# Graphegon/pygraphblas

Measured on AMD Instinct MI355X. Metric: GFLOPS + GB/s (vs roofline) for mxv/mxm on R-MAT-22, 1/2/4/8 GPU, higher is better.
Workload: dtype f64; 1 GPU; R-MAT scale-22 FP64 PLUS_TIMES SpMV (GrB_mxv), edgefactor 16, BASELINE.json configs[1]; n=4194304, nnz=65245211, semiring=PLUS_TIMES_FP64, parallelism=rowblock1, transport=none (one GPU), device=AMD Radeon Graphics gfx950:sramecc+:xnack-

## Files before the change

### pygraphblas_amd/csrc/grb_spmv_xcd.hpp

```cpp
#pragma once
#include "grb_spmv_tiles.hpp"
#include "grb_matops.hpp"

namespace grb {

constexpr int XP = 8;
constexpr int XPMAX = 64;
constexpr uint32_t XP_RB = 1024;
constexpr int XP_CT = 512;
constexpr uint32_t XP_UNIT = 16384;
constexpr int XP_ST = 512;
constexpr int XP_SW = XP_ST / 64;

struct XcdPlan {
  DevBuf hot_cols;
  DevBuf pcol, pval;
  DevBuf trow;
  DevBuf col16, extras, tinfo;
  uint64_t ncold = 0;
  DevBuf lrow;
  DevBuf blockptr;
  DevBuf m_bstart;
  DevBuf m_blockptr;
  DevBuf m_slot;
// ... 264 lines not shown
    const uint2 hh = *(const uint2*)(col16 + q0);
    const uint32_t h[2] = {hh.x, hh.y};
    uint32_t before = 0, nc = 0;
    for (int u = 0; u < 4; u++) {
      const uint32_t w = (h[u >> 1] >> (16 * (u & 1))) & 0x7FFFu; const bool cold = w >= H;
      const unsigned long long m = __ballot(cold);
      before += __builtin_amdgcn_mbcnt_hi((uint32_t)(m >> 32), __builtin_amdgcn_mbcnt_lo((uint32_t)m, 0u)); nc += cold ? 1u : 0u;
    }
    const uint32_t xr = tinfo[2 * (size_t)g + 1] + before;
    uint32_t x0 = 0, x1 = 0, x2 = 0;
    if (nc) { const uint32_t* xp = (const uint32_t*)extras + (xr >> 1); x0 = xp[0]; x1 = xp[1]; x2 = xp[2]; }
    const uint64_t wa = ((uint64_t)x1 << 32) | x0, wb = ((uint64_t)x2 << 32) | x1;
    uint32_t q = xr & 1u;
    for (int u = 0; u < 4; u++) {
      const uint32_t w16 = (h[u >> 1] >> (16 * (u & 1))) & 0xFFFFu, code = w16 & 0x7FFFu, flag = (w16 & 0x8000u) << 16;
      const bool cold = code >= H;
      const uint32_t lo = (uint32_t)((q < 2u ? wa >> (16u * q) : wb >> (16u * (q - 2u)))) & 0xFFFFu;
      const uint32_t c = flag | (cold ? XT_COLD | (((code - H) << 16) | lo) : code);
      q += cold ? 1u : 0u;
      if (c != pcol[q0 + u]) { const unsigned long long n = atomicAdd(bad, 1ull); if (n == 0) { bad[1] = q0 + u; bad[2] = ((unsigned long long)c << 32) | pcol[q0 + u]; } }
    }
    if (lane == 0 && tinfo[2 * (size_t)g] != trow[g]) atomicAdd(bad + 3, 1ull);
  }
}
template <class T> __global__ __launch_bounds__(256) void k_xp_hot_gather(const T* __restrict__ u, const uint32_t* __restrict__ hot_cols, uint32_t total, T* __restrict__ xhot) {
  for (uint32_t i = (blockIdx.x * 256 + threadIdx.x) * 4u; i < total; i += gridDim.x * 1024u) {
    if (i + 4u <= total) {
      const uint4 c = *(const uint4*)(hot_cols + i);
      const T x0 = u[c.x], x1 = u[c.y], x2 = u[c.z], x3 = u[c.w];
      xhot[i] = x0; xhot[i + 1] = x1; xhot[i + 2] = x2; xhot[i + 3] = x3;
    } else for (uint32_t j = i; j < total; j++) xhot[j] = u[hot_cols[j]];
  }
}
constexpr uint32_t XP_CONT = 0x8000u, XP_HEAD = 0x4000u, XP_LROW = 0x07FFu;
static_assert(XP_RB <= XP_LROW + 1, "row id inside a block and the two flags share 16 bits");
static __global__ void k_xp_cont_flags(const uint32_t* __restrict__ subrow_row, const uint32_t* __restrict__ vfirst, uint16_t* __restrict__ lrow) {
  uint32_t pb[XP + 1];
#pragma unroll
  for (int k = 0; k <= XP; k++) pb[k] = vfirst[k];
  const uint32_t F = pb[XP];
  for (uint32_t s = blockIdx.x * 256 + threadIdx.x; s < F; s += gridDim.x * 256) {
    const uint32_t r = subrow_row[s];
    bool first = false, last = s + 1 == F;
#pragma unroll
    for (int k = 0; k <= XP; k++) { first = first || pb[k] == s; last = last || pb[k] == s + 1; }
    const bool cont = !first && subrow_row[s - 1] == r, more = !last && subrow_row[s + 1] == r;
    lrow[s] = (uint16_t)((r % XP_RB) | (cont ? XP_CONT : 0u) | (!cont && more ? XP_HEAD : 0u));
  }
}
constexpr int XP_NA = 2;
template <class T, class SR>
__global__ __launch_bounds__(XP_CT) void k_xp_combine(uint32_t nrows, const uint32_t* __restrict__ blockptr, const uint16_t* __restrict__ subrow_lrow, const T* __restrict__ partial,
                                                      T* __restrict__ y, uint8_t* __restrict__ ypres, const SR sr) {
  __shared__ T acc[XP_NA][XP_RB];
  __shared__ uint8_t has[XP_NA][XP_RB];
  __shared__ T cval[2][XP_NA][XP_CT];
  __shared__ uint8_t ccont[2][XP_NA][XP_CT + 1];
  const uint32_t b = blockIdx.x, r0 = b * XP_RB, tid = threadIdx.x;
  for (uint32_t i = tid; i < XP_NA * XP_RB; i += XP_CT) (&has[0][0])[i] = 0;
  if (tid < 2 * XP_NA) ccont[tid / XP_NA][tid % XP_NA][XP_CT] = 0;
  uint32_t lo[XP], hi[XP], longest = 0;
#pragma unroll
  for (int k = 0; k < XP; k++) { lo[k] = blockptr[b * XP + k]; hi[k] = blockptr[(b + 1) * XP + k]; longest = hi[k] - lo[k] > longest ? hi[k] - lo[k] : longest; }
  for (uint32_t base = 0; base < longest; base += XP_CT) {
    uint32_t w[XP]; T v[XP];
#pragma unroll
    for (int k = 0; k < XP; k++) {
      const uint32_t s = lo[k] + base + tid; const bool ok = s < hi[k];
      w[k] = ok ? (uint32_t)subrow_lrow[s] : XP_CONT; v[k] = ok ? partial[s] : T();
    }
#pragma unroll
    for (int k0 = 0; k0 < XP; k0 += XP_NA) {
      const int buf = (k0 / XP_NA) & 1;
#pragma unroll
      for (int j = 0; j < XP_NA; j++) {
        const int k = k0 + j;
        const bool cont = (w[k] & XP_CONT) != 0 && lo[k] + base + tid < hi[k];
        ccont[buf][j][tid] = cont ? 1 : 0;
        if (cont) cval[buf][j][tid] = v[k];
      }
      __syncthreads();
#pragma unroll
      for (int j = 0; j < XP_NA; j++) {
        const int k = k0 + j;
        if (!(w[k] & XP_CONT)) {
          const uint32_t r = w[k] & XP_LROW; T x = v[k];
          const bool h = has[j][r] != 0; const T a = acc[j][r];
          if (w[k] & XP_HEAD) {
            uint32_t q = tid + 1;
            while (ccont[buf][j][q]) { x = sr.add(x, cval[buf][j][q]); q++; }
            if (q == XP_CT) for (uint32_t g = lo[k] + base + XP_CT; g < hi[k] && (subrow_lrow[g] & XP_CONT); g++) x = sr.add(x, partial[g]);
          }
          acc[j][r] = h ? sr.add(a, x) : x; has[j][r] = 1;
        }
      }
    }
    __syncthreads();
  }
  __syncthreads();
  for (uint32_t i = tid; i < XP_RB; i += XP_CT) {
    const uint32_t r = r0 + i;
    if (r < nrows) {
      bool h = has[0][i] != 0; T x = acc[0][i];
#pragma unroll
      for (int j = 1; j < XP_NA; j++) { const bool hj = has[j][i] != 0; const T xj = acc[j][i]; x = h ? (hj ? sr.add(x, xj) : x) : xj; h = h || hj; }
      y[r] = h ? x : T(); ypres[r] = h ? 1 : 0;
    }
  }
}

constexpr uint32_t XM_ROWS = 1024, XM_TARGET = 2048, XM_SLOTS = 2560;
constexpr int XM_CT = 256;
#ifndef XM_INFL
#define XM_INFL 4
#endif
static __global__ void k_xm_iota(uint32_t* p, uint64_t n) { for (uint64_t i = blockIdx.x * 256ull + threadIdx.x; i < n; i += gridDim.x * 256ull) p[i] = (uint32_t)i; }
static __global__ void k_xm_weights(const uint32_t* __restrict__ cnt, uint32_t nrows, uint32_t perrow, uint32_t* __restrict__ w) {
  for (uint32_t r = blockIdx.x * 256 + threadIdx.x; r <= nrows; r += gridDim.x * 256) w[r] = r < nrows ? cnt[r] + perrow : 0u;
}
static __global__ void k_xm_newblock(const uint32_t* __restrict__ P, uint32_t nrows, uint32_t target, uint32_t* __restrict__ f) {
  for (uint32_t r = blockIdx.x * 256 + threadIdx.x; r <= nrows; r += gridDim.x * 256) f[r] = r < nrows && (r == 0 || P[r] / target != P[r - 1] / target) ? 1u : 0u;
}
static __global__ void k_xm_bstart(const uint32_t* __restrict__ f, const uint32_t* __restrict__ fscan, uint32_t nrows, uint32_t nblocks, uint32_t* __restrict__ bstart) {
  for (uint32_t r = blockIdx.x * 256 + threadIdx.x; r <= nrows; r += gridDim.x * 256) { if (r == nrows) bstart[nblocks] = nrows; else if (f[r]) bstart[fscan[r]] = r; }
}
static __global__ void k_xm_rowoff(const uint32_t* __restrict__ f, const uint32_t* __restrict__ fscan, const uint32_t* __restrict__ bstart, const uint32_t* __restrict__ rfirst, uint32_t nrows,
                                   uint16_t* __restrict__ rowoff) {
  for (uint32_t r = blockIdx.x * 256 + threadIdx.x; r < nrows; r += gridDim.x * 256) { const uint32_t b = fscan[r] + f[r] - 1; rowoff[r] = (uint16_t)(rfirst[r] - rfirst[bstart[b]]); }
}
static __global__ void k_xm_slots(const uint32_t* __restrict__ skey, const uint32_t* __restrict__ sidx, uint64_t F, const uint32_t* __restrict__ f, const uint32_t* __restrict__ fscan,
                                  const uint32_t* __restrict__ bstart, const uint32_t* __restrict__ rfirst, uint16_t* __restrict__ slot) {
  for (uint64_t i = blockIdx.x * 256ull + threadIdx.x; i < F; i += gridDim.x * 256ull) { const uint32_t r = skey[i], b = fscan[r] + f[r] - 1; slot[sidx[i]] = (uint16_t)((uint32_t)i - rfirst[bstart[b]]); }
}
static __global__ void k_xm_block_starts(const uint32_t* __restrict__ subrow_row, const uint32_t* __restrict__ bstart, uint32_t nblocks, const uint32_t* __restrict__ vfirst, uint32_t np,
                                         uint32_t* __restrict__ blockptr) {
  for (uint32_t t = blockIdx.x * 256 + threadIdx.x; t < (nblocks + 1) * np; t += gridDim.x * 256) {
    const uint32_t b = t / np, k = t % np; const uint32_t target = bstart[b];
    uint32_t lo = vfirst[k], hi = vfirst[k + 1];
    while (lo < hi) { const uint32_t mid = lo + ((hi - lo) >> 1); if (subrow_row[mid] < target) lo = mid + 1; else hi = mid; }
    blockptr[t] = lo;
  }
}
static __global__ void k_xm_max(const uint32_t* __restrict__ cnt, uint32_t nrows, uint32_t* __restrict__ out) {
  __shared__ uint32_t s_m;
  if (threadIdx.x == 0) s_m = 0;
  __syncthreads();
  uint32_t m = 0;
  for (uint32_t r = blockIdx.x * 256 + threadIdx.x; r < nrows; r += gridDim.x * 256) m = cnt[r] > m ? cnt[r] : m;
  m = __builtin_amdgcn_wave_reduce_max_u32(m, 0);
  if ((threadIdx.x & 63) == 0 && m) atomicMax(&s_m, m);
  __syncthreads();
  if (threadIdx.x == 0 && s_m) atomicMax(out, s_m);
}
template <class T, class SR, int EPI = 0>
__global__ __launch_bounds__(XM_CT) void k_xp_merge(uint32_t nrows, uint32_t nblocks, const uint32_t* __restrict__ bstart, const uint32_t* __restrict__ blockptr, const uint16_t* __restrict__ slot,
                                                    const uint16_t* __restrict__ rowoff, const T* __restrict__ partial, T* __restrict__ y, uint8_t* __restrict__ ypres, const SR sr, const T fill = T()) {
  extern __shared__ __attribute__((aligned(16))) unsigned char xm_lds[];
  T* const vals = (T*)xm_lds;
  const uint32_t per = gridDim.x / XP, b = (blockIdx.x & (XP - 1)) * per + (blockIdx.x >> 3);
  const uint32_t tid = threadIdx.x;
  if (b >= nblocks) return;
  const uint32_t r0 = bstart[b], r1 = bstart[b + 1];
  uint32_t lo[XP], pre[XP + 1];
  pre[0] = 0;
#pragma unroll
  for (int k = 0; k < XP; k++) { lo[k] = blockptr[b * XP + k]; pre[k + 1] = pre[k] + (blockptr[(b + 1) * XP + k] - lo[k]); }
  const uint32_t total = pre[XP];
  for (uint32_t t0 = tid; t0 < total; t0 += XM_INFL * XM_CT) {
    T v[XM_INFL]; uint32_t sl[XM_INFL];
#pragma unroll
    for (int u = 0; u < XM_INFL; u++) {
      const uint32_t t = t0 + u * XM_CT; const bool ok = t < total;
      uint32_t s = 0;
#pragma unroll
      for (int k = 0; k < XP; k++) if (t >= pre[k] && t < pre[k + 1]) s = lo[k] + (t - pre[k]);
      v[u] = ok ? partial[s] : T(); sl[u] = ok ? (uint32_t)slot[s] : 0xFFFFFFFFu;
    }
#pragma unroll
    for (int u = 0; u < XM_INFL; u++) if (sl[u] != 0xFFFFFFFFu) vals[sl[u]] = v[u];
  }
  __syncthreads();
  const int lane = tid & 63;
  const uint32_t nr = r1 - r0, nround = (nr + XM_CT - 1) / XM_CT * XM_CT;
  for (uint32_t i = tid; i < nround; i += XM_CT) {
    const bool live = i < nr;
    const uint32_t r = r0 + i;
    const uint32_t o0 = live ? (uint32_t)rowoff[r] : 0u, o1 = live ? (i + 1 < nr ? (uint32_t)rowoff[r + 1] : total) : 0u;
    const bool wide = o1 - o0 > 64u;
    T acc = T();
    if (o1 > o0 && !wide) { acc = vals[o0]; for (uint32_t q = o0 + 1; q < o1; q++) acc = sr.add(acc, vals[q]); }
    unsigned long long todo = __ballot(wide);
    while (todo) {
      const int L = __builtin_ctzll(todo); todo &= todo - 1;
      const uint32_t q0 = (uint32_t)__shfl((int)o0, L, 64), q1 = (uint32_t)__shfl((int)o1, L, 64);
      T part = sr.identity; bool has = false;
      for (uint32_t q = q0 + lane; q < q1; q += 64) { part = has ? sr.add(part, vals[q]) : vals[q]; has = true; }
      const T red = wave_reduce_op<T, false>(sr.add_op(), has ? part : sr.identity);
      if (lane == L) acc = red;
    }
    if constexpr (EPI == 0) { if (live) { y[r] = acc; ypres[r] = o1 > o0 ? 1 : 0; } }
    else if constexpr (EPI == 1) { if (live && o1 > o0) y[r] = sr.add(y[r], acc); }
    else if constexpr (EPI == 2) { if (live) { y[r] = o1 > o0 ? sr.add(fill, acc) : fill; ypres[r] = 1; } }
    else {
      if constexpr (std::is_arithmetic<T>::value) {
        if (live && o1 > o0 && (sr.add_op() == B_MIN ? acc < fill : acc > fill)) { if (ypres[r]) y[r] = sr.add(y[r], acc); else { y[r] = acc; ypres[r] = 1; } }
      }
    }
  }
}

#ifndef XMW_TARGET_V
#define XMW_TARGET_V 4096
#endif
constexpr uint32_t XMW_TARGET = XMW_TARGET_V, XMW_ROWS = XMW_TARGET_V / 2;
constexpr int XMW_RPT = XMW_ROWS / XM_CT;
template <class T, class SR, int EPI = 0>
__global__ __launch_bounds__(XM_CT) void k_xp_merge_wide(uint32_t nrows, uint32_t nblocks, const uint32_t* __restrict__ bstart, const uint32_t* __restrict__ blockptr, const uint16_t* __restrict__ slot,
                                                         const uint16_t* __restrict__ rowoff, const T* __restrict__ partial, T* __restrict__ y, uint8_t* __restrict__ ypres, const SR sr, const T fill,
                                                         const uint32_t np, const uint32_t m_slots) {
  extern __shared__ __attribute__((aligned(16))) unsigned char xm_lds[];
  T* const vals = (T*)xm_lds;
  uint8_t* const flag = xm_lds + (size_t)m_slots * sizeof(T);
  __shared__ uint32_t s_lo[XPMAX], s_pre[XPMAX + 1];
  __shared__ T s_tsum[XM_CT];
  __shared__ uint8_t s_hasflag[XM_CT];
  const uint32_t per = (nblocks + XP - 1) / XP, tid = threadIdx.x, stride = gridDim.x >> 3;
  auto block_of = [&](uint32_t bb) -> uint32_t { const uint32_t b = (blockIdx.x & (XP - 1)) * per + bb; return bb < per && b < nblocks ? b : 0xFFFFFFFFu; };
  uint32_t bb = blockIdx.x >> 3, b = block_of(bb);
  uint32_t n_r0 = 0, n_r1 = 0, n_l0 = 0, n_len = 0;
  auto fetch_bounds = [&](uint32_t bn) __attribute__((always_inline)) {
    if (bn == 0xFFFFFFFFu) return;
    n_r0 = bstart[bn]; n_r1 = bstart[bn + 1];
    if (tid < np) { n_l0 = blockptr[bn * np + tid]; n_len = blockptr[(bn + 1) * np + tid] - n_l0; }
  };
  fetch_bounds(b);
  for (; b != 0xFFFFFFFFu; ) {
  __syncthreads();
  const uint32_t r0 = n_r0, r1 = n_r1, nr = r1 - r0;
  if (tid < 64u) {
    const bool in = tid < np;
    const uint32_t l0 = in ? n_l0 : 0u, len = in ? n_len : 0u;
    uint32_t incl = len;
#pragma unroll
    for (int d = 1; d < 64; d <<= 1) { const uint32_t o = (uint32_t)__shfl_up((int)incl, d, 64); if ((int)tid >= d) incl += o; }
    s_lo[tid] = l0; s_pre[tid] = in ? incl - len : 0xFFFFFFFFu;
    if (tid == 63u) { if (np < 64u) s_pre[np] = incl; s_pre[XPMAX] = np < 64u ? 0xFFFFFFFFu : incl; }
  }
  for (uint32_t q = tid * 4u; q < m_slots; q += XM_CT * 4u) *(uint32_t*)(flag + q) = 0u;
  uint32_t o0[XMW_RPT], o1[XMW_RPT];
#pragma unroll
  for (int j = 0; j < XMW_RPT; j++) {
    const uint32_t i = tid + (uint32_t)j * XM_CT; const bool live = i < nr;
    o0[j] = live ? (uint32_t)rowoff[r0 + i] : 0u;
    o1[j] = live && i + 1 < nr ? (uint32_t)rowoff[r0 + i + 1] : 0u;
  }
  __syncthreads();
  const uint32_t total = s_pre[np];
  bb += stride; const uint32_t b_next = block_of(bb);
  fetch_bounds(b_next);
  auto run_of = [&](uint32_t t) __attribute__((always_inline)) -> uint32_t {
    uint32_t k = 0;
#pragma unroll
    for (uint32_t step = 32u; step; step >>= 1) { const uint32_t cand = k + step; k = s_pre[cand] <= t ? cand : k; }
    return k;
  };
  for (uint32_t base = 0; base < total; base += 2u * XM_CT * 4u) {
    T v[2][4]; uint32_t sl[2][4];
#pragma unroll
    for (int g = 0; g < 2; g++) {
      const uint32_t t = base + (tid + (uint32_t)g * XM_CT) * 4u;
      uint32_t src[4]; bool ok[4];
      uint32_t k = t < total ? run_of(t) : 0u;
      uint32_t base = s_lo[k] - s_pre[k], end = s_pre[k + 1];
#pragma unroll
      for (int e = 0; e < 4; e++) {
        const uint32_t te = t + (uint32_t)e; ok[e] = te < total;
        while (ok[e] && te >= end) { k++; base = s_lo[k] - s_pre[k]; end = s_pre[k + 1]; }
        src[e] = ok[e] ? base + te : 0u;
      }
#pragma unroll
      for (int e = 0; e < 4; e++) { v[g][e] = ok[e] ? partial[src[e]] : T(); sl[g][e] = ok[e] ? (uint32_t)slot[src[e]] : 0xFFFFFFFFu; }
    }
#pragma unroll
    for (int g = 0; g < 2; g++)
#pragma unroll
      for (int e = 0; e < 4; e++) if (sl[g][e] != 0xFFFFFFFFu) vals[sl[g][e]] = v[g][e];
  }
#pragma unroll
  for (int j = 0; j < XMW_RPT; j++) {
    const uint32_t i = tid + (uint32_t)j * XM_CT;
    if (i < nr && i + 1 == nr) o1[j] = total;
    if (i < nr && o1[j] > o0[j]) flag[o0[j]] = 1;
  }
  __syncthreads();
  const uint32_t chunk = ((total + XM_CT - 1) / XM_CT) | 1u;
  const uint32_t q0 = tid * chunk < total ? tid * chunk : total, q1 = q0 + chunk < total ? q0 + chunk : total;
  uint32_t first = WP_NONE;
  {
    T acc = sr.identity;
    for (uint32_t q = q0; q < q1; q++) {
      const T v = vals[q]; const bool f = flag[q] != 0;
      acc = f ? v : sr.add(acc, v);
      vals[q] = acc;
      first = f && first == WP_NONE ? q : first;
    }
    s_tsum[tid] = acc; s_hasflag[tid] = first != WP_NONE ? 1 : 0;
  }
  __syncthreads();
  {
    const uint32_t lead_end = first != WP_NONE ? first : q1;
    const bool ends_row = lead_end == total || flag[lead_end < total ? lead_end : 0u] != 0;
    if (q1 > q0 && first != q0 && ends_row) {
      T c = sr.identity;
      for (uint32_t t = tid; t > 0;) { t--; c = sr.add(s_tsum[t], c); if (s_hasflag[t]) break; }
      vals[lead_end - 1u] = sr.add(c, vals[lead_end - 1u]);
    }
  }
  __syncthreads();
#pragma unroll
  for (int j = 0; j < XMW_RPT; j++) {
    const uint32_t i = tid + (uint32_t)j * XM_CT;
    if (i < nr) {
      const uint32_t r = r0 + i;
      const bool has = o1[j] > o0[j]; const T acc = has ? vals[o1[j] - 1u] : T();
      if constexpr (EPI == 0) { y[r] = acc; ypres[r] = has ? 1 : 0; }
      else if constexpr (EPI == 1) { if (has) y[r] = sr.add(y[r], acc); }
      else if constexpr (EPI == 2) { y[r] = has ? sr.add(fill, acc) : fill; ypres[r] = 1; }
      else {
        if constexpr (std::is_arithmetic<T>::value) {
          if (has && (sr.add_op() == B_MIN ? acc < fill : acc > fill)) { if (ypres[r]) y[r] = sr.add(y[r], acc); else { y[r] = acc; ypres[r] = 1; } }
        }
      }
    }
  }
  b = b_next;
  }
}

struct XtVariant { int depth, waves, exp; };
inline XtVariant xt_variant() {
  XtVariant v{XT_DEPTH, XT_WAVES, 0};
#ifdef XT_VARIANTS
  const char* e = getenv("GRB_MI355X_XT");
  if (e) { int d = v.depth, w = v.waves, x = 0; if (sscanf(e, "d%dw%de%d", &d, &w, &x) >= 2) { v.depth = d; v.waves = w; v.exp = x; } }
#endif
  return v;
}

template <class T> int xp_subpanels(uint64_t ncols, bool* forced_out) {
  const uint32_t forced = wp_env("GRB_MI355X_XS", 0);
  *forced_out = forced == 1 || forced == 2 || forced == 4 || forced == 8;
  if (*forced_out) return (int)forced;
  if (sizeof(T) <= 4 && ncols >= (1ull << 25)) return 8;
  if (ncols >= (1ull << 24)) return 4;
  if (sizeof(T) <= 4 && ncols >= (1ull << 23)) return 2;
  return 1;
}
static __global__ void k_xp_neg(const uint32_t* __restrict__ cnt, uint32_t n, uint32_t* __restrict__ key) {
// ... 224 lines not shown
    }
    gr.cbase[NS] = nchunks;
    DevBuf lc(((size_t)nchunks + 1) * 4), cstep(((size_t)nchunks + 1) * 4), pk((XPMAX + 2) * 4);
    GRB_HIP(hipMemsetAsync(lc.as<uint32_t>() + nchunks, 0, 4, stream()));
    { unsigned nb = (nchunks + 3) / 4; if (nb < 1) nb = 1; if (nb > 16384) nb = 16384;
      hipLaunchKernelGGL(k_sell_lc, dim3(nb), dim3(256), 0, stream(), sorted.as<uint32_t>(), plen.as<uint32_t>(), gr, nchunks, lc.as<uint32_t>()); }
    exclusive_scan_u32(lc.as<uint32_t>(), cstep.as<uint32_t>(), (uint64_t)nchunks + 1);
    hipLaunchKernelGGL(k_sell_pick, dim3(1), dim3(128), 0, stream(), cstep.as<uint32_t>(), gr, pk.as<uint32_t>());
    uint32_t hs[XPMAX + 2];
    GRB_HIP(hipMemcpyAsync(hs, pk.p, (NS + 1) * 4, hipMemcpyDeviceToHost, stream())); GRB_HIP(hipStreamSynchronize(stream()));
    const uint64_t nsteps = hs[NS];
    if (nsteps && nsteps * 256ull < (1ull << 40)) {
      P->s_nsteps = nsteps; P->s_nchunks = nchunks;
      P->s_col.alloc(nsteps * 256 + 64); P->s_perm.alloc((size_t)nchunks * 256 + 64);
      GRB_HIP(hipMemsetAsync(P->s_col.p, 0, nsteps * 256 + 64, stream())); GRB_HIP(hipMemsetAsync(P->s_perm.p, 0xFF, (size_t)nchunks * 256 + 64, stream()));
      if (with_vals) { P->s_val.alloc(nsteps * 64 * sizeof(T) + 64); GRB_HIP(hipMemsetAsync(P->s_val.p, 0, nsteps * 64 * sizeof(T) + 64, stream())); }
      hipLaunchKernelGGL(k_sell_inv, dim3(grid_n(F)), dim3(256), 0, stream(), sorted.as<uint32_t>(), F, inv.as<uint32_t>());
      hipLaunchKernelGGL((k_sell_scatter<T>), dim3(tile_grid), dim3(256), 0, stream(), P->pcol.as<uint32_t>(), with_vals ? P->pval.as<T>() : (const T*)nullptr, E.as<uint32_t>(), pstart.as<uint32_t>(),
                         inv.as<uint32_t>(), lc.as<uint32_t>(), cstep.as<uint32_t>(), sst, gr, ntiles, P->s_col.as<uint32_t>(), with_vals ? P->s_val.as<T>() : (T*)nullptr, P->s_perm.as<uint32_t>());
      { unsigned nb = (nchunks + 3) / 4; if (nb < 1) nb = 1; if (nb > 16384) nb = 16384;
        hipLaunchKernelGGL(k_sell_meta, dim3(nb), dim3(256), 0, stream(), P->s_col.as<uint32_t>(), lc.as<uint32_t>(), cstep.as<uint32_t>(), gr, nchunks); }
      uint32_t ibase[XPMAX + 1], nitems = 0;
      for (uint32_t k = 0; k < NS; k++) { ibase[k] = nitems; nitems += (hs[k + 1] - hs[k] + SELL_ITEM - 1) / SELL_ITEM; }
      ibase[NS] = nitems; P->s_nitems = nitems;
      DevBuf dib((XPMAX + 1) * 4);
      GRB_HIP(hipMemcpyAsync(dib.p, ibase, (NS + 1) * 4, hipMemcpyHostToDevice, stream()));
      P->s_items.alloc(((size_t)nitems + 2) * 4);
      hipLaunchKernelGGL(k_sell_items, dim3(grid_n((uint64_t)nitems + 1)), dim3(256), 0, stream(), cstep.as<uint32_t>(), gr, dib.as<uint32_t>(), nitems, (uint32_t)nsteps, P->s_items.as<uint32_t>());
      memcpy(sell_hs, hs, sizeof(uint32_t) * (NS + 1)); memcpy(sell_ib, ibase, sizeof(uint32_t) * (NS + 1));
      GRB_HIP(hipStreamSynchronize(stream()));
      P->sell = true;
      if (getenv("GRB_MI355X_VERBOSE")) fprintf(stderr, "[grb] lane-per-piece layout: %llu pieces in %u chunks, %llu steps = %.3f x the entries, %u work items\n", (unsigned long long)F, nchunks,
                                                (unsigned long long)nsteps, (double)nsteps * 64.0 / (double)nnz, nitems);
    }
  }
  constexpr bool c16 = xt_fmt<T>::C16;
  const bool keep32 = !c16 || wp_env("GRB_MI355X_XT_KEEP32", 0) != 0;
  if (c16) {
    DevBuf tcnt(((size_t)ntiles + 1) * 4), tcold(((size_t)ntiles + 1) * 4);
    GRB_HIP(hipMemsetAsync(tcnt.as<uint32_t>() + ntiles, 0, 4, stream()));
    unsigned nb = (ntiles + 3) / 4; if (nb < 1) nb = 1; if (nb > 16384) nb = 16384;
    hipLaunchKernelGGL(k_xc_count, dim3(nb), dim3(256), 0, stream(), P->pcol.as<uint32_t>(), ntiles, H, tcnt.as<uint32_t>());
    exclusive_scan_u32(tcnt.as<uint32_t>(), tcold.as<uint32_t>(), (uint64_t)ntiles + 1);
    uint32_t nc32 = 0;
    GRB_HIP(hipMemcpyAsync(&nc32, tcold.as<uint32_t>() + ntiles, 4, hipMemcpyDeviceToHost, stream())); GRB_HIP(hipStreamSynchronize(stream()));
    P->ncold = nc32;
    P->col16.alloc(nstore * 2); P->extras.alloc(P->ncold * 2 + 32); P->tinfo.alloc(((size_t)ntiles + 1) * 8);
    hipLaunchKernelGGL(k_xc_pack, dim3(nb), dim3(256), 0, stream(), P->pcol.as<uint32_t>(), P->trow.as<uint32_t>(), tcold.as<uint32_t>(), ntiles, H, P->col16.as<uint16_t>(), P->extras.as<uint16_t>(),
                       P->tinfo.as<uint32_t>());
    if (wp_env("GRB_MI355X_XC_VERIFY", 0)) {
      DevBuf bad(64); GRB_HIP(hipMemsetAsync(bad.p, 0, 64, stream()));
      hipLaunchKernelGGL(k_xc_verify, dim3(nb), dim3(256), 0, stream(), P->pcol.as<uint32_t>(), P->col16.as<uint16_t>(), P->extras.as<uint16_t>(), P->tinfo.as<uint32_t>(), P->trow.as<uint32_t>(), ntiles, H,
                         (unsigned long long*)bad.p);
      unsigned long long hb[4]; GRB_HIP(hipMemcpyAsync(hb, bad.p, 32, hipMemcpyDeviceToHost, stream())); GRB_HIP(hipStreamSynchronize(stream()));
      fprintf(stderr, "[grb] 16-bit column plane check: %llu words differ (first at entry %llu: decoded %08llx, stored %08llx), %llu tile infos differ; cold entries %llu of %llu\n", hb[0], hb[1], hb[2] >> 32,
              hb[2] & 0xFFFFFFFFull, hb[3], (unsigned long long)P->ncold, (unsigned long long)nstore);
    }
    if (!keep32) { P->pcol.reset(); P->trow.reset(); }
  }
  P->vbytes = (int)sizeof(T);
  if constexpr (std::is_integral<T>::value && (sizeof(T) == 4 || sizeof(T) == 8)) {
    if (with_vals && !P->sell && wp_env("GRB_MI355X_XT_NARROW", 1) != 0) {
      DevBuf flag(64); GRB_HIP(hipMemsetAsync(flag.p, 0, 64, stream()));
      const unsigned g = (unsigned)std::min<uint64_t>((nstore + 255) / 256, 4096);
      hipLaunchKernelGGL((k_xt_fits16<T>), dim3(g), dim3(256), 0, stream(), P->pval.as<T>(), (uint64_t)nstore, flag.as<uint32_t>());
      uint32_t hf = 1; GRB_HIP(hipMemcpyAsync(&hf, flag.p, 4, hipMemcpyDeviceToHost, stream())); GRB_HIP(hipStreamSynchronize(stream()));
      if (hf == 0) {
        DevBuf narrow(nstore * 2 + 64);
        hipLaunchKernelGGL((k_xt_narrow16<T>), dim3(g), dim3(256), 0, stream(), P->pval.as<T>(), (uint64_t)nstore, narrow.as<int16_t>());
        P->pval = std::move(narrow); P->vbytes = 2;
      }
    }
  }
  P->args.alloc(XPMAX * sizeof(XtPanel<T>));
  P->xhot.alloc((size_t)NS * H * sizeof(T) + 8); P->partial.alloc(P->F * sizeof(T) + 8);
  XtPanel<T> ha[XPMAX];
  memset((void*)ha, 0, sizeof(ha));
  for (uint32_t k = 0; k < NS; k++) {
    XtPanel<T>& a = ha[k];
    a.pcol = keep32 ? P->pcol.as<uint32_t>() + (size_t)P->tbase[k] * WP_ENT : nullptr; a.aval = with_vals ? (const T*)((const char*)P->pval.p + (size_t)P->tbase[k] * WP_ENT * (size_t)P->vbytes) : nullptr;
    a.trow = keep32 ? P->trow.as<uint32_t>() + P->tbase[k] : nullptr; a.xhot = P->xhot.as<T>() + (size_t)k * H;
    a.col16 = c16 ? P->col16.as<uint16_t>() + (size_t)P->tbase[k] * WP_ENT : nullptr; a.tinfo = c16 ? P->tinfo.as<uint32_t>() + 2 * (size_t)P->tbase[k] : nullptr;
    a.extras = c16 ? P->extras.as<uint16_t>() : nullptr; a.nextras = P->ncold;
    a.nnz = (uint32_t)P->ne[k]; a.ntiles = P->ntiles[k]; a.tiles_per_chunk = kt[k]; a.nhot = P->nhot[k];
    a.static_pct = wp_env("GRB_MI355X_WP_STATIC", WP_STATIC_PCT);
    a.interleave = wp_env("GRB_MI355X_XT_INTERLEAVE", vps > 1 ? 1u : 0u);
  }
  if (getenv("GRB_MI355X_VERBOSE"))
    for (uint32_t k = 0; k < NS; k++)
      fprintf(stderr, "[grb] xcd plan stream %u: entries %llu tiles %u chunk %u hot %u (sub-rows in all %llu, chunks %llu, sub-panels per XCD %d, %s)\n", k, (unsigned long long)P->ne[k], P->ntiles[k], kt[k],
              P->nhot[k], (unsigned long long)P->F, (unsigned long long)nchunks_total, S, own ? "a table per sub-panel" : "a table per XCD");
  GRB_HIP(hipMemcpyAsync(P->args.p, ha, sizeof(ha), hipMemcpyHostToDevice, stream()));
  SellPanel<T> sa[XPMAX]; memset((void*)sa, 0, sizeof(sa));
  if (P->sell) {
    for (uint32_t k = 0; k < NS; k++) {
      SellPanel<T>& a = sa[k];
      a.scol = P->s_col.as<uint32_t>() + (size_t)sell_hs[k] * 64; a.sval = with_vals ? P->s_val.as<T>() + (size_t)sell_hs[k] * 64 : nullptr;
      a.item_first = P->s_items.as<uint32_t>() + sell_ib[k]; a.step0 = sell_hs[k]; a.nsteps = sell_hs[k + 1] - sell_hs[k]; a.nitems = sell_ib[k + 1] - sell_ib[k];
      a.xhot = P->xhot.as<T>() + (size_t)k * H; a.nhot = P->nhot[k];
      a.static_pct = wp_env("GRB_MI355X_WP_STATIC", WP_STATIC_PCT); a.interleave = wp_env("GRB_MI355X_XT_INTERLEAVE", vps > 1 ? 1u : 0u);
    }
    P->s_args.alloc(sizeof(sa));
    GRB_HIP(hipMemcpyAsync(P->s_args.p, sa, sizeof(sa), hipMemcpyHostToDevice, stream()));
  }
  P->tsize = (int)sizeof(T); P->has_vals = with_vals;
  GRB_HIP(hipEventRecord(ev1, stream()));
  GRB_HIP(hipStreamSynchronize(stream()));
  GRB_HIP(hipEventElapsedTime(&P->build_ms, ev0, ev1)); g_xcd_plan_build_ms = P->build_ms;
  (void)hipEventDestroy(ev0); (void)hipEventDestroy(ev1);
}

template <class T> bool run_xcd(const SpmvCall& c, const SemiringDesc& d, int ncu) {
  DevCSR& M = *c.M;
  if (ncu < XP || ncu % XP) return false;
  if ((uint64_t)M.ncols > xt_hot<T>::MAXCOLS) return false;
  const bool need_vals = c.aval != nullptr;
  if (need_vals && c.aval != M.val.p) return false;
  auto* P = static_cast<XcdPlan*>(M.xcd.get());
  if (!P || P->tsize != (int)sizeof(T) || (need_vals && !P->has_vals)) { build_xcd_plan<T>(M, ncu, need_vals); P = static_cast<XcdPlan*>(M.xcd.get()); }
  const bool uses_u = d.flip ? binop_uses_x(d.mulop) : binop_uses_y(d.mulop);
  constexpr uint32_t H = xt_hot<T>::H;
  XtCall<T> call{(const T*)c.uval, M.ncols, (uint32_t)(P->NS / XP), P->partial.as<T>()};
  if (uses_u) hipLaunchKernelGGL((k_xp_hot_gather<T>), dim3(((uint32_t)P->NS * H + 1023) / 1024), dim3(256), 0, stream(), (const T*)c.uval, P->hot_cols.as<uint32_t>(), (uint32_t)P->NS * H, P->xhot.as<T>());
  with_semiring<T>(d, [&](auto sr) {
    typedef decltype(sr) SR;
    bool launched = false;
#ifdef XT_VARIANTS
    if constexpr (std::is_same<SR, StaticSR<double, B_PLUS, B_TIMES>>::value) {
      const XtVariant v = xt_variant();
#define XT_TRY(D_, W_, E_) if (!launched && v.depth == D_ && v.waves == W_ && v.exp == E_) { \
        hipLaunchKernelGGL((k_spmv_tiles<T, SR, D_, W_, E_>), dim3(ncu), dim3(W_ * 64), 0, stream(), call, (const XtPanel<T>*)P->args.p, sr); launched = true; }
      XT_TRY(1, 16, 1) XT_TRY(1, 16, 2) XT_TRY(2, 16, 0)
      if (!launched && v.exp == 4 && ((const XcdPlan*)P)->pcol.p) {
        hipLaunchKernelGGL((k_spmv_tiles<T, SR, XT_DEPTH, XT_WAVES, 0, false>), dim3(ncu), dim3(XT_WAVES * 64), 0, stream(), call, (const XtPanel<T>*)P->args.p, sr); launched = true; } XT_TRY(1, 8, 0) XT_TRY(2, 8, 0) XT_TRY(3, 8, 0) XT_TRY(2, 8, 2) XT_TRY(3, 8, 2) XT_TRY(4, 8, 0)
#undef XT_TRY
    }
#endif
    if constexpr (sizeof(T) == 4 || sizeof(T) == 8) {
      const bool sell_off = wp_env("GRB_MI355X_SELL_RUN", 1) == 0;
      if (!launched && P->sell && !sell_off) {
        hipLaunchKernelGGL((k_spmv_sell<T, SR>), dim3(ncu), dim3(XT_WAVES * 64), 0, stream(), call, (const SellPanel<T>*)P->s_args.p, P->s_perm.as<uint32_t>(), P->s_nchunks, sr);
        launched = true;
      }
    }
    if constexpr (std::is_integral<T>::value && (sizeof(T) == 4 || sizeof(T) == 8)) {
      if (!launched && P->vbytes == 2) {
        hipLaunchKernelGGL((k_spmv_tiles<T, SR, XT_DEPTH, XT_WAVES, 0, xt_fmt<T>::C16, 2>), dim3(ncu), dim3(XT_WAVES * 64), 0, stream(), call, (const XtPanel<T>*)P->args.p, sr);
        launched = true;
      }
    }
    if (!launched) hipLaunchKernelGGL((k_spmv_tiles<T, SR>), dim3(ncu), dim3(XT_WAVES * 64), 0, stream(), call, (const XtPanel<T>*)P->args.p, sr);
    const uint32_t nblocks = (uint32_t)(((uint64_t)M.nrows + XP_RB - 1) / XP_RB);
    static const bool old_merge = wp_env("GRB_MI355X_XP_OLD_MERGE", 0) != 0;
    if (P->m_ok && (!old_merge || P->m_wide)) {
      const dim3 mg((P->m_nblocks + XP - 1) / XP * XP), mb(XM_CT); const size_t ml = (size_t)P->m_slots * sizeof(T);
      const uint32_t np = (uint32_t)P->NP;
      static const uint32_t wg_per_cu = wp_env("GRB_MI355X_XMW_WGS", 6);
      const dim3 mgw(std::min<uint32_t>(mg.x, (uint32_t)ncu * wg_per_cu / XP * XP));
#define XM_LAUNCH(EPI_, Y_, YP_, FILL_) { \
        if (P->m_wide) hipLaunchKernelGGL((k_xp_merge_wide<T, SR, EPI_>), mgw, mb, ml + P->m_slots, stream(), M.nrows, P->m_nblocks, P->m_bstart.as<uint32_t>(), P->m_blockptr.as<uint32_t>(), \
                                         P->m_slot.as<uint16_t>(), P->m_rowoff.as<uint16_t>(), P->partial.as<T>(), (Y_), (YP_), sr, (FILL_), np, P->m_slots); \
        else hipLaunchKernelGGL((k_xp_merge<T, SR, EPI_>), mg, mb, ml, stream(), M.nrows, P->m_nblocks, P->m_bstart.as<uint32_t>(), P->m_blockptr.as<uint32_t>(), P->m_slot.as<uint16_t>(), \
                                P->m_rowoff.as<uint16_t>(), P->partial.as<T>(), (Y_), (YP_), sr, (FILL_)); }
      if (c.epi == 1 && c.epi_done) {
        XM_LAUNCH(1, (T*)c.epi_w, (uint8_t*)nullptr, T())
        *c.epi_done = true;
      } else if (c.epi == 2 && c.epi_done) {
        T fill; memcpy(&fill, c.epi_fill, sizeof(T));
        XM_LAUNCH(2, (T*)c.tval, c.tpres, fill)
        *c.epi_done = true;
      } else if (c.epi == 3 && c.epi_done && std::is_arithmetic<T>::value) {
        T th; memcpy(&th, c.epi_fill, sizeof(T));
        XM_LAUNCH(3, (T*)c.epi_w, c.epi_wpres, th)
        *c.epi_done = true;
      } else XM_LAUNCH(0, (T*)c.tval, c.tpres, T())
#undef XM_LAUNCH
    } else
      hipLaunchKernelGGL((k_xp_combine<T, SR>), dim3(nblocks), dim3(XP_CT), 0, stream(), M.nrows, P->blockptr.as<uint32_t>(), P->lrow.as<uint16_t>(), P->partial.as<T>(),
                         (T*)c.tval, c.tpres, sr);
    g_last_plan += std::string("k_spmv_xcd<") + (sr.is_static ? "static" : "dynamic") + (P->sell ? ",lane-per-piece" : "") + (P->vbytes == 2 && P->has_vals ? ",values=int16" : "") + ",subrows=" + std::to_string(P->F) + (P->S > 1 ? ",subpanels=" + std::to_string(P->S) + (P->own ? "/own-tables" : "") : std::string()) + "," + xcd_mapping() + "> ";
  });
  return true;
}

}
```

Before: 534.8 GFLOP/s.

## Restructure XCD merge kernel with buffer loads, hoisted offsets and blocked row stores

Rewrites the non-wide merge kernel of the XCD SpMV. Block metadata is read through scalar constant loads, and the per-partial source index is computed with precomputed deltas instead of a compare chain. Partials and slots are fetched with bounds-checked buffer loads in one deep batch per thread. Row offsets are loaded before the scatter barrier so their latency overlaps, and each thread now owns a contiguous run of rows so y and ypres can be written as vector stores. The trade-offs are more register pressure, 32-bit buffer addressing (guarded by a new size check at launch), and a behaviour that depends on XM_CHAIN compile flags.

```diff
diff --git a/pygraphblas_amd/csrc/grb_spmv_xcd.hpp b/pygraphblas_amd/csrc/grb_spmv_xcd.hpp
--- a/pygraphblas_amd/csrc/grb_spmv_xcd.hpp
+++ b/pygraphblas_amd/csrc/grb_spmv_xcd.hpp
@@ -440,58 +440,114 @@
   __syncthreads();
   if (threadIdx.x == 0 && s_m) atomicMax(out, s_m);
 }
+#ifndef XM_CHAIN
+#define XM_CHAIN 15
+#endif
+constexpr int XM_PAIRS = (XM_CHAIN & 4) ? (int)(XM_SLOTS / XM_CT) : XM_INFL;
+constexpr int XM_RPT = (int)XM_ROWS / XM_CT;
 template <class T, class SR, int EPI = 0>
 __global__ __launch_bounds__(XM_CT) void k_xp_merge(uint32_t nrows, uint32_t nblocks, const uint32_t* __restrict__ bstart, const uint32_t* __restrict__ blockptr, const uint16_t* __restrict__ slot,
-                                                    const uint16_t* __restrict__ rowoff, const T* __restrict__ partial, T* __restrict__ y, uint8_t* __restrict__ ypres, const SR sr, const T fill = T()) {
+                                                    const uint16_t* __restrict__ rowoff, const T* __restrict__ partial, T* __restrict__ y, uint8_t* __restrict__ ypres, const SR sr, const T fill,
+                                                    const uint32_t F) {
   extern __shared__ __attribute__((aligned(16))) unsigned char xm_lds[];
   T* const vals = (T*)xm_lds;
   const uint32_t per = gridDim.x / XP, b = (blockIdx.x & (XP - 1)) * per + (blockIdx.x >> 3);
   const uint32_t tid = threadIdx.x;
   if (b >= nblocks) return;
-  const uint32_t r0 = bstart[b], r1 = bstart[b + 1];
-  uint32_t lo[XP], pre[XP + 1];
+  uint32_t r0, r1, pre[XP + 1], dl[XP];
   pre[0] = 0;
-#pragma unroll
-  for (int k = 0; k < XP; k++) { lo[k] = blockptr[b * XP + k]; pre[k + 1] = pre[k] + (blockptr[(b + 1) * XP + k] - lo[k]); }
-  const uint32_t total = pre[XP];
-  for (uint32_t t0 = tid; t0 < total; t0 += XM_INFL * XM_CT) {
-    T v[XM_INFL]; uint32_t sl[XM_INFL];
-#pragma unroll
-    for (int u = 0; u < XM_INFL; u++) {
-      const uint32_t t = t0 + u * XM_CT; const bool ok = t < total;
-      uint32_t s = 0;
-#pragma unroll
-      for (int k = 0; k < XP; k++) if (t >= pre[k] && t < pre[k + 1]) s = lo[k] + (t - pre[k]);
-      v[u] = ok ? partial[s] : T(); sl[u] = ok ? (uint32_t)slot[s] : 0xFFFFFFFFu;
-    }
-#pragma unroll
-    for (int u = 0; u < XM_INFL; u++) if (sl[u] != 0xFFFFFFFFu) vals[sl[u]] = v[u];
+  if constexpr ((XM_CHAIN & 1) != 0) {
+    const XT_K uint32_t* const kb = (const XT_K uint32_t*)(uintptr_t)bstart + b;
+    const XT_K uint32_t* const kp = (const XT_K uint32_t*)(uintptr_t)blockptr + (size_t)b * XP;
+    r0 = kb[0]; r1 = kb[1];
+#pragma unroll
+    for (int k = 0; k < XP; k++) { const uint32_t lo = kp[k]; pre[k + 1] = pre[k] + (kp[XP + k] - lo); dl[k] = lo - pre[k]; }
+  } else {
+    r0 = bstart[b]; r1 = bstart[b + 1];
+#pragma unroll
+    for (int k = 0; k < XP; k++) { const uint32_t lo = blockptr[b * XP + k]; pre[k + 1] = pre[k] + (blockptr[(b + 1) * XP + k] - lo); dl[k] = lo - pre[k]; }
+  }
+  const uint32_t total = pre[XP], nr = r1 - r0;
+  uint32_t o0[XM_RPT], o1[XM_RPT];
+  auto row_of = [&](int j) -> uint32_t { return (XM_CHAIN & 8) ? tid * (uint32_t)XM_RPT + (uint32_t)j : tid + (uint32_t)j * XM_CT; };
+  auto load_offsets = [&]() __attribute__((always_inline)) {
+    const __amdgpu_buffer_rsrc_t o_rsrc = __builtin_amdgcn_make_buffer_rsrc((void*)(rowoff + r0), (short)0, (int)(nr * 2u), 0x00020000);
+    if constexpr ((XM_CHAIN & 8) != 0) {
+      uint32_t e[XM_RPT + 1];
+#pragma unroll
+      for (int j = 0; j <= XM_RPT; j++) e[j] = (uint32_t)xt_buf_load<uint16_t>(o_rsrc, (tid * (uint32_t)XM_RPT + (uint32_t)j) * 2u);
+#pragma unroll
+      for (int j = 0; j < XM_RPT; j++) { o0[j] = e[j]; o1[j] = e[j + 1]; }
+    } else {
+#pragma unroll
+      for (int j = 0; j < XM_RPT; j++) { o0[j] = (uint32_t)xt_buf_load<uint16_t>(o_rsrc, row_of(j) * 2u); o1[j] = (uint32_t)xt_buf_load<uint16_t>(o_rsrc, row_of(j) * 2u + 2u); }
+    }
+  };
+  if constexpr ((XM_CHAIN & 2) != 0) load_offsets();
+  const __amdgpu_buffer_rsrc_t p_rsrc = __builtin_amdgcn_make_buffer_rsrc((void*)partial, (short)0, (int)(F * (uint32_t)sizeof(T)), 0x00020000);
+  const __amdgpu_buffer_rsrc_t s_rsrc = __builtin_amdgcn_make_buffer_rsrc((void*)slot, (short)0, (int)(F * 2u), 0x00020000);
+  for (uint32_t base = 0; base < total; base += XM_PAIRS * XM_CT) {
+    T v[XM_PAIRS]; uint32_t sl[XM_PAIRS];
+#pragma unroll
+    for (int u = 0; u < XM_PAIRS; u++) {
+      const uint32_t t = base + tid + u * XM_CT; const bool ok = t < total;
+      uint32_t d = dl[0];
+#pragma unroll
+      for (int k = 1; k < XP; k++) d = t >= pre[k] ? dl[k] : d;
+      const uint32_t s = t + d;
+      if constexpr ((XM_CHAIN & 4) != 0) { v[u] = xt_buf_load<T>(p_rsrc, ok ? s * (uint32_t)sizeof(T) : 0xFFFFFFFFu); sl[u] = (uint32_t)xt_buf_load<uint16_t>(s_rsrc, ok ? s * 2u : 0xFFFFFFFFu); }
+      else { v[u] = ok ? partial[s] : T(); sl[u] = ok ? (uint32_t)slot[s] : 0u; }
+    }
+#pragma unroll
+    for (int u = 0; u < XM_PAIRS; u++) if (base + tid + u * XM_CT < total) vals[sl[u]] = v[u];
   }
   __syncthreads();
+  if constexpr ((XM_CHAIN & 2) == 0) load_offsets();
   const int lane = tid & 63;
-  const uint32_t nr = r1 - r0, nround = (nr + XM_CT - 1) / XM_CT * XM_CT;
-  for (uint32_t i = tid; i < nround; i += XM_CT) {
-    const bool live = i < nr;
-    const uint32_t r = r0 + i;
-    const uint32_t o0 = live ? (uint32_t)rowoff[r] : 0u, o1 = live ? (i + 1 < nr ? (uint32_t)rowoff[r + 1] : total) : 0u;
-    const bool wide = o1 - o0 > 64u;
-    T acc = T();
-    if (o1 > o0 && !wide) { acc = vals[o0]; for (uint32_t q = o0 + 1; q < o1; q++) acc = sr.add(acc, vals[q]); }
+  T acc[XM_RPT]; bool has[XM_RPT];
+#pragma unroll
+  for (int j = 0; j < XM_RPT; j++) {
+    const uint32_t i = row_of(j); const bool live = i < nr;
+    o1[j] = live ? (i + 1 < nr ? o1[j] : total) : 0u; o0[j] = live ? o0[j] : 0u;
+    const uint32_t q0 = o0[j], q1 = o1[j];
+    const bool wide = q1 - q0 > 64u;
+    T a = T();
+    if (q1 > q0 && !wide) { a = vals[q0]; for (uint32_t q = q0 + 1; q < q1; q++) a = sr.add(a, vals[q]); }
     unsigned long long todo = __ballot(wide);
     while (todo) {
       const int L = __builtin_ctzll(todo); todo &= todo - 1;
-      const uint32_t q0 = (uint32_t)__shfl((int)o0, L, 64), q1 = (uint32_t)__shfl((int)o1, L, 64);
-      T part = sr.identity; bool has = false;
-      for (uint32_t q = q0 + lane; q < q1; q += 64) { part = has ? sr.add(part, vals[q]) : vals[q]; has = true; }
-      const T red = wave_reduce_op<T, false>(sr.add_op(), has ? part : sr.identity);
-      if (lane == L) acc = red;
-    }
-    if constexpr (EPI == 0) { if (live) { y[r] = acc; ypres[r] = o1 > o0 ? 1 : 0; } }
-    else if constexpr (EPI == 1) { if (live && o1 > o0) y[r] = sr.add(y[r], acc); }
-    else if constexpr (EPI == 2) { if (live) { y[r] = o1 > o0 ? sr.add(fill, acc) : fill; ypres[r] = 1; } }
+      const uint32_t w0 = (uint32_t)__shfl((int)q0, L, 64), w1 = (uint32_t)__shfl((int)q1, L, 64);
+      T part = sr.identity; bool any = false;
+      for (uint32_t q = w0 + lane; q < w1; q += 64) { part = any ? sr.add(part, vals[q]) : vals[q]; any = true; }
+      const T red = wave_reduce_op<T, false>(sr.add_op(), any ? part : sr.identity);
+      if (lane == L) a = red;
+    }
+    acc[j] = a; has[j] = q1 > q0;
+  }
+  if constexpr ((XM_CHAIN & 8) != 0 && (EPI == 0 || EPI == 2)) {
+    const uint32_t i0 = tid * (uint32_t)XM_RPT;
+    if (i0 + XM_RPT <= nr) {
+      T out[XM_RPT]; uint8_t pb[XM_RPT];
+#pragma unroll
+      for (int j = 0; j < XM_RPT; j++) {
+        if constexpr (EPI == 0) { out[j] = acc[j]; pb[j] = has[j] ? 1 : 0; }
+        else { out[j] = has[j] ? sr.add(fill, acc[j]) : fill; pb[j] = 1; }
+      }
+      __builtin_memcpy((void*)(y + (size_t)r0 + i0), out, sizeof(out));
+      __builtin_memcpy((void*)(ypres + (size_t)r0 + i0), pb, sizeof(pb));
+      return;
+    }
+  }
+#pragma unroll
+  for (int j = 0; j < XM_RPT; j++) {
+    const uint32_t i = row_of(j), r = r0 + i;
+    if (i >= nr) continue;
+    if constexpr (EPI == 0) { y[r] = acc[j]; ypres[r] = has[j] ? 1 : 0; }
+    else if constexpr (EPI == 1) { if (has[j]) y[r] = sr.add(y[r], acc[j]); }
+    else if constexpr (EPI == 2) { y[r] = has[j] ? sr.add(fill, acc[j]) : fill; ypres[r] = 1; }
     else {
       if constexpr (std::is_arithmetic<T>::value) {
-        if (live && o1 > o0 && (sr.add_op() == B_MIN ? acc < fill : acc > fill)) { if (ypres[r]) y[r] = sr.add(y[r], acc); else { y[r] = acc; ypres[r] = 1; } }
+        if (has[j] && (sr.add_op() == B_MIN ? acc[j] < fill : acc[j] > fill)) { if (ypres[r]) y[r] = sr.add(y[r], acc[j]); else { y[r] = acc[j]; ypres[r] = 1; } }
       }
     }
   }
@@ -1022,7 +1078,7 @@
     if (!launched) hipLaunchKernelGGL((k_spmv_tiles<T, SR>), dim3(ncu), dim3(XT_WAVES * 64), 0, stream(), call, (const XtPanel<T>*)P->args.p, sr);
     const uint32_t nblocks = (uint32_t)(((uint64_t)M.nrows + XP_RB - 1) / XP_RB);
     static const bool old_merge = wp_env("GRB_MI355X_XP_OLD_MERGE", 0) != 0;
-    if (P->m_ok && (!old_merge || P->m_wide)) {
+    if (P->m_ok && (P->m_wide || (!old_merge && (uint64_t)P->F * sizeof(T) < (1ull << 32)))) {
       const dim3 mg((P->m_nblocks + XP - 1) / XP * XP), mb(XM_CT); const size_t ml = (size_t)P->m_slots * sizeof(T);
       const uint32_t np = (uint32_t)P->NP;
       static const uint32_t wg_per_cu = wp_env("GRB_MI355X_XMW_WGS", 6);
@@ -1031,7 +1087,7 @@
         if (P->m_wide) hipLaunchKernelGGL((k_xp_merge_wide<T, SR, EPI_>), mgw, mb, ml + P->m_slots, stream(), M.nrows, P->m_nblocks, P->m_bstart.as<uint32_t>(), P->m_blockptr.as<uint32_t>(), \
                                          P->m_slot.as<uint16_t>(), P->m_rowoff.as<uint16_t>(), P->partial.as<T>(), (Y_), (YP_), sr, (FILL_), np, P->m_slots); \
         else hipLaunchKernelGGL((k_xp_merge<T, SR, EPI_>), mg, mb, ml, stream(), M.nrows, P->m_nblocks, P->m_bstart.as<uint32_t>(), P->m_blockptr.as<uint32_t>(), P->m_slot.as<uint16_t>(), \
-                                P->m_rowoff.as<uint16_t>(), P->partial.as<T>(), (Y_), (YP_), sr, (FILL_)); }
+                                P->m_rowoff.as<uint16_t>(), P->partial.as<T>(), (Y_), (YP_), sr, (FILL_), (uint32_t)P->F); }
       if (c.epi == 1 && c.epi_done) {
         XM_LAUNCH(1, (T*)c.epi_w, (uint8_t*)nullptr, T())
         *c.epi_done = true;
```

Result: no change. 530.8 GFLOP/s (-0.7%).
